# sebadorn/Physically-based-Rendering

Hardware: AMD Instinct MI355X
Metric: Msamples/s (paths/s) @1080p fixed seed; 1/2/4/8 MI355X scaling (higher is better)
Workload: dtype f32

## Files before the change

### physically-based-rendering_amd/csrc/pbr_hip.hip

```cpp
#include <hip/hip_runtime.h>

#include <cmath>
#include <cstdarg>
#include <cstdio>
#include <cstdlib>
#include <cstring>
#include <string>
#include <algorithm>
#include <vector>

#include "pbr_hip.h"
#include "pbr_hip_diag.h"
#include "pt_aux.hpp"
#include "pt_adaptive.hpp"
#include "pt_instances.hpp"
#include "bvh_build.hpp"
#include "pt_denoise.hpp"
#include "pt_scene_pack.hpp"
#include "pt_tuner.hpp"
#include "pt_adaptive_host.hpp"

using ptk::DevParams;

typedef void ( *KernelFn )( const ptk::DevParams );
// ... 91 lines not shown
	bool plansBuilt = false, phongPlanBuilt = false, chainPlansBuilt = false;
	bool workClean = false;
	float* hSeeds = nullptr;
	size_t hSeedCapacity = 0;
	int pinnedPlan = -1;
	char lastPlan[48] = "";
	char lastKernel[96] = "";
	double lastTraceMs = 0.0;
	uint32_t lastTraceLaunches = 0;
	float* dSeeds = nullptr;
	size_t seedCapacity = 0;
	unsigned long long* dCounters = nullptr;
	unsigned int* dWork = nullptr;
	unsigned int* dGuard = nullptr;
	unsigned* dTileFrames = nullptr;
	float* dTileError = nullptr;
	unsigned* dTileActive = nullptr;
	float2* dMoments = nullptr;
	unsigned* dAdaptiveOrder = nullptr;
	hipEvent_t evFoldStart = nullptr, evFoldStop = nullptr;
	bool adaptiveStats = false;
	uint32_t lastAdaptiveRounds = 0;
	uint64_t lastAdaptiveUnits = 0;
	double lastAdaptiveFoldMs = 0.0;
};

namespace {

int fail( pbr_ctx* ctx, int code, const char* fmt, ... ) {
	char buf[512];
	va_list ap;
	va_start( ap, fmt );
	vsnprintf( buf, sizeof( buf ), fmt, ap );
	va_end( ap );

	if( ctx != nullptr ) {
		ctx->error = buf;
	}

	return code;
}

#define HIP_TRY( ctx, call ) \
	do { \
		const hipError_t err__ = ( call ); \
		if( err__ != hipSuccess ) { \
			return fail( ctx, PBR_EDEVICE, "%s: %s", #call, hipGetErrorString( err__ ) ); \
		} \
	} while( 0 )

#define PBR_TRY( call ) \
	do { \
		const int status__ = ( call ); \
		if( status__ != PBR_OK ) { \
			return status__; \
		} \
	} while( 0 )

void freeWalkStreams( pbr_ctx* ctx ) {
	(void) hipFree( ctx->dNodesWalk );
	ctx->dNodesWalk = nullptr;
	ctx->walkBuilt = 0;
	ctx->walkBytes = 0;
}

void freeScene( pbr_ctx* ctx ) {
	(void) hipFree( ctx->dNodes );
	freeWalkStreams( ctx );
	(void) hipFree( ctx->dTris );
	(void) hipFree( ctx->dTriPN );
	ctx->dTriPN = nullptr;
	(void) hipFree( ctx->dFaceN );
	ctx->dFaceN = nullptr;
	(void) hipFree( ctx->dMats );
	(void) hipFree( ctx->dLights );
	ctx->dNodes = ctx->dTris = ctx->dMats = ctx->dLights = nullptr;
	ctx->hasScene = false;
}

void replan( pbr_ctx* ctx ) {
	ctx->plansBuilt = false;
	ctx->chainPlansBuilt = false;
	ctx->phongPlanBuilt = false;
	ctx->tuner.reset( ScheduleTuner::scaleOf( (size_t) ctx->numLocalTiles * 64 ) );
}

void freeImages( pbr_ctx* ctx ) {
	(void) hipFree( ctx->dImgIn );
	(void) hipFree( ctx->dImgOut );
	(void) hipFree( ctx->dImgDbg );
	(void) hipFree( ctx->dRows );
	(void) hipFree( ctx->dFull );
	(void) hipFree( ctx->dFrameBuf );
	ctx->dFrameBuf = nullptr;
	ctx->frameBufFrames = 0;
	(void) hipFree( ctx->dChain );
	ctx->dChain = nullptr;
	ctx->chainFloats = 0;
	(void) hipFree( ctx->dTileOrder );
	(void) hipFree( ctx->dCostOrder );
	(void) hipFree( ctx->dLastOrder );
	ctx->dLastOrder = nullptr;
	ctx->hLastOrder.clear();
	(void) hipFree( ctx->dTileCost );
	(void) hipFree( ctx->dTileFrames );
	(void) hipFree( ctx->dTileError );
	(void) hipFree( ctx->dTileActive );
	(void) hipFree( ctx->dMoments );
	(void) hipFree( ctx->dAdaptiveOrder );
	ctx->dTileFrames = ctx->dTileActive = ctx->dAdaptiveOrder = nullptr;
	ctx->dTileError = nullptr;
	ctx->dMoments = nullptr;
	ctx->adaptiveStats = false;
	ctx->dTileOrder = ctx->dCostOrder = nullptr;
	ctx->dTileCost = nullptr;
	ctx->hTileOrder.clear();
	ctx->hCostOrder.clear();
	ctx->costLearnt = false;
	ctx->orderPinned = false;
	ctx->dImgIn = ctx->dImgOut = ctx->dImgDbg = ctx->dRows = ctx->dFull = nullptr;
	ctx->configured = false;
}

const size_t kWorkBytes = sizeof( unsigned int ) * ( PT_HEADS + 1 ) * PT_BAND_STRIDE;

const size_t kFrameBufBytes = (size_t) 16 << 30;

const size_t kCounterSlots = 16;


#define PTI_DECLARE( f, g ) extern "C" const void* PTI_NAME( f, g )( uint32_t, int, int ) __attribute__( ( weak ) );
#define PTI_DECLARE_FLAVOUR( f ) \
	PTI_DECLARE( f, 0 ) PTI_DECLARE( f, 1 ) PTI_DECLARE( f, 2 ) PTI_DECLARE( f, 3 ) PTI_DECLARE( f, 4 ) PTI_DECLARE( f, 5 ) PTI_DECLARE( f, 6 ) PTI_DECLARE( f, 7 ) \
	PTI_DECLARE( f, 8 )
PTI_DECLARE_FLAVOUR( 0 )
PTI_DECLARE_FLAVOUR( 1 )
PTI_DECLARE_FLAVOUR( 2 )
PTI_DECLARE_FLAVOUR( 3 )
PTI_DECLARE_FLAVOUR( 5 )
PTI_DECLARE_FLAVOUR( 7 )
PTI_DECLARE_FLAVOUR( 8 )
PTI_DECLARE_FLAVOUR( 9 )
PTI_DECLARE_FLAVOUR( 10 )
PTI_DECLARE_FLAVOUR( 11 )
PTI_DECLARE_FLAVOUR( 13 )
PTI_DECLARE_FLAVOUR( 15 )
#define PTI_ROW( f ) { PTI_NAME( f, 0 ), PTI_NAME( f, 1 ), PTI_NAME( f, 2 ), PTI_NAME( f, 3 ), PTI_NAME( f, 4 ), PTI_NAME( f, 5 ), PTI_NAME( f, 6 ), PTI_NAME( f, 7 ), PTI_NAME( f, 8 ) }
#define PTI_NO_ROW { nullptr, nullptr, nullptr, nullptr, nullptr, nullptr, nullptr, nullptr, nullptr }
const pti_picker kPickers[PTI_FLAVOURS][PTI_GROUPS] = { PTI_ROW( 0 ), PTI_ROW( 1 ), PTI_ROW( 2 ), PTI_ROW( 3 ), PTI_NO_ROW, PTI_ROW( 5 ), PTI_NO_ROW, PTI_ROW( 7 ),
                                                       PTI_ROW( 8 ), PTI_ROW( 9 ), PTI_ROW( 10 ), PTI_ROW( 11 ), PTI_NO_ROW, PTI_ROW( 13 ), PTI_NO_ROW, PTI_ROW( 15 ) };

KernelFn pickKernel( int flavour, int group, uint32_t brdf, bool shadow, bool lights ) {
	const pti_picker pick = kPickers[flavour][group];
	return ( pick != nullptr ) ? (KernelFn) pick( brdf, shadow ? 1 : 0, lights ? 1 : 0 ) : nullptr;
}

int flavourOf( uint32_t traversal, uint32_t arith ) {
	return ( ( traversal != 0 ) ? 1 : 0 ) | ( ( arith != 0 ) ? 2 : 0 ) | ( ( traversal == PBR_WALK_EIGHT_ORDERS_COMPACT ) ? 4 : 0 );
}

int flavourOf( const pbr_config& cfg ) {
	return flavourOf( cfg.traversal, cfg.arith );
}

bool dualIsDual( int flavour );

// ... 309 lines not shown
	const size_t slotBytes = spec.pathSlotBytes;

	if( share < slotBytes + 32 ) {
		return fail( ctx, PBR_ESTATE, "plan %s: %zu B of per-lane path state do not fit a block's %zu B share of LDS at %d blocks per CU", spec.name, slotBytes, share, blocksPerCU );
	}

	size_t slots = ( share - slotBytes ) / 32;
	slots = std::min<size_t>( slots, hotAvail );

	if( knobs.ldsSlots >= 0 ) {
		slots = std::min<size_t>( slots, (size_t) knobs.ldsSlots );
	}
	if( flavour & 4 ) {
		slots &= ~(size_t) 1;
	}

	HIP_TRY( ctx, hipFuncSetAttribute( (const void*) kernel, hipFuncAttributeMaxDynamicSharedMemorySize, (int) share ) );

	plan->kernel = kernel;
	plan->blockThreads = spec.blockThreads;
	plan->blocks = ctx->numCUs * blocksPerCU;
	plan->numHot = (int) slots;
	plan->ldsBytes = slots * 32 + slotBytes;
	plan->park = spec.park;
	plan->shade = spec.shade;
	plan->parkEighths = ( ctx->numNodes >= kWideMinNodes ) ? 4 : 6;
	plan->refillBatch = ( knobs.refillBatch >= 1 ) ? std::min( 64, knobs.refillBatch ) : ( ( ctx->numNodes >= kWideMinNodes ) ? kRefillBatchLarge : kRefillBatchSmall );
	plan->drainMode = ( knobs.drainMode >= 0 ) ? knobs.drainMode : 1;

	if( knobs.phPark >= 0 ) {
		plan->park = std::max( 1, std::min( ( spec.pathSlotBytes != 0 ) ? 128 : 64, knobs.phPark ) );
	}
	if( knobs.phShade >= 0 ) {
		plan->shade = std::max( 1, std::min( 64, knobs.phShade ) );
	}
	if( knobs.parkEighths >= 0 ) {
		plan->parkEighths = std::min( 8, knobs.parkEighths );
	}

	plan->name = spec.name;
	const char* const tf[2] = { "false", "true" };
	const int minw[PTI_GROUPS] = { 4, 6, 8, 4, 4, 6, 8, 0, 0 };

	if( spec.group == PTI_DUAL ) {
		std::snprintf( plan->kernelName, sizeof( plan->kernelName ), "ptk_f%d::pathTracingDual<%u, %s, %s>", flavour, ctx->cfg.brdf, tf[shadow], tf[lights] );
	}
	else if( spec.group >= PTI_PHASED_LEAN ) {
		std::snprintf( plan->kernelName, sizeof( plan->kernelName ), "ptk_f%d::pathTracingPhased<%u, %s, %s, %d>", flavour, ctx->cfg.brdf, tf[shadow], tf[lights], minw[spec.group] );
	}
	else {
		std::snprintf( plan->kernelName, sizeof( plan->kernelName ), "ptk_f%d::pathTracing<%u, %s, %s, %d, %s>", flavour, ctx->cfg.brdf, tf[shadow], tf[lights], minw[spec.group], tf[spec.group == PTI_REFILL_PHONG] );
	}

	return PBR_OK;
}

int buildPlans( pbr_ctx* ctx, uint32_t hotAvail, bool phong, bool chained ) {
	if( !ctx->plansBuilt || ( chained && !ctx->chainPlansBuilt ) ) {
		const int flavour = flavourOf( ctx->cfg );
		const bool orderedWalk = ( flavour & 1 ) != 0;
		const PlanSpec specs[ScheduleTuner::kPlans] = {
			{ PTI_REFILL_LEAN, "refill-lean", 0, 0 },
			{ PTI_REFILL_WIDE, "refill-wide", 0, 0 },
			{ PTI_PHASED_LEAN, "phased-lean", 16, 32 },
			{ PTI_PHASED_WIDE, "phased-wide", 16, 48 },
			{ PTI_PHASED_MID, "phased-mid", orderedWalk ? 12 : 16, orderedWalk ? 48 : 40, kMidBlockThreads },
			{ PTI_REFILL_MID, "refill-mid", 0, 0, kMidBlockThreads },
			dualIsDual( flavour ) ? PlanSpec{ PTI_DUAL, "phased-dual", 28, 48, PBR_BLOCK, (size_t) 2 * 4 * 16 * PBR_BLOCK }
			                      : PlanSpec{ PTI_PHASED_MID, "phased-dual", 16, 40, kMidBlockThreads },
		};

		for( int k = 0; k < ScheduleTuner::kPlans; k++ ) {
			if( !ctx->plansBuilt ) {
				PBR_TRY( makePlan( ctx, specs[k], hotAvail, &ctx->plans[k] ) );
				ctx->tuner.names[k] = specs[k].name;
			}
			if( chained && !ctx->chainPlansBuilt ) {
				PBR_TRY( makePlan( ctx, specs[k], hotAvail, &ctx->chainPlans[k], true ) );
			}
		}

		ctx->chainPlansBuilt = ctx->chainPlansBuilt || chained;

		ctx->tuner.log = ( ctx->knobs.tuneLog > 0 ) ? stderr : nullptr;
		ctx->phongPlanBuilt = ctx->plansBuilt && ctx->phongPlanBuilt;
		ctx->plansBuilt = true;
	}

	if( phong && !ctx->phongPlanBuilt ) {
		PBR_TRY( makePlan( ctx, PlanSpec{ PTI_REFILL_PHONG, "refill-lean-phong", 0, 0 }, hotAvail, &ctx->phongPlan ) );
		ctx->phongPlanBuilt = true;
	}

	return PBR_OK;
}

int runPlan( pbr_ctx* ctx, const Plan& plan, DevParams* P, size_t waveUnits ) {
	const size_t wavesPerBlock = (size_t) plan.blockThreads / 64;
	const size_t needed = std::max<size_t>( 1, ( waveUnits + wavesPerBlock - 1 ) / wavesPerBlock );
	const unsigned blocks = (unsigned) std::min<size_t>( (size_t) plan.blocks, needed );
	P->numHot = plan.numHot;
	P->numHotBytes = plan.numHot * 32;
	P->slotBase = plan.numHot * 32;
	P->phPark = plan.park;
	P->phShade = plan.shade;
	P->refillBatch = plan.refillBatch;
	P->drainMode = plan.drainMode;
	P->parkEighths = plan.parkEighths;
	hipLaunchKernelGGL( plan.kernel, dim3( blocks ), dim3( (unsigned) plan.blockThreads ), plan.ldsBytes, ctx->stream, *P );
	HIP_TRY( ctx, hipGetLastError() );
	return PBR_OK;
}

int stageSeeds( pbr_ctx* ctx, const float* seeds, uint32_t nFrames ) {
	if( ctx->seedCapacity < nFrames ) {
		(void) hipFree( ctx->dSeeds );
		ctx->dSeeds = nullptr;
		ctx->seedCapacity = 0;
		HIP_TRY( ctx, hipMalloc( (void**) &ctx->dSeeds, sizeof( float ) * nFrames ) );
		ctx->seedCapacity = nFrames;
	}

	if( ctx->hSeedCapacity < nFrames ) {
		(void) hipHostFree( ctx->hSeeds );
		ctx->hSeeds = nullptr;
		ctx->hSeedCapacity = 0;
		HIP_TRY( ctx, hipHostMalloc( (void**) &ctx->hSeeds, sizeof( float ) * std::max<size_t>( nFrames, 64 ), hipHostMallocDefault ) );
		ctx->hSeedCapacity = std::max<size_t>( nFrames, 64 );
	}

	std::memcpy( ctx->hSeeds, seeds, sizeof( float ) * nFrames );
	HIP_TRY( ctx, hipMemcpyAsync( ctx->dSeeds, ctx->hSeeds, sizeof( float ) * nFrames, hipMemcpyHostToDevice, ctx->stream ) );
	return PBR_OK;
}

int growFrameBuf( pbr_ctx* ctx, uint32_t nFrames, size_t* chunkCap ) {
	const size_t pixelSlots = (size_t) ctx->numLocalTiles * 64;
	const size_t frameBytes = sizeof( float4 ) * pixelSlots;
	const size_t capFrames = std::max<size_t>( 1, kFrameBufBytes / frameBytes );
	size_t cap = std::min<size_t>( capFrames, nFrames );
	cap = std::min<size_t>( cap, std::max<size_t>( 1, 0x7FFFFFFFull / ( pixelSlots + 64 * (size_t) ctx->queueWidth ) ) );

	if( ctx->knobs.chunkFrames >= 1 ) {
		cap = std::min<size_t>( cap, (size_t) ctx->knobs.chunkFrames );
	}

	*chunkCap = cap;

	if( ctx->frameBufFrames < cap ) {
		const size_t frames = std::min<size_t>( capFrames, std::max<size_t>( 256, ( cap <= 256 ) ? cap : 2 * cap ) );
		(void) hipFree( ctx->dFrameBuf );
		ctx->dFrameBuf = nullptr;
		ctx->frameBufFrames = 0;
		HIP_TRY( ctx, hipMalloc( (void**) &ctx->dFrameBuf, frameBytes * frames ) );
		ctx->frameBufFrames = frames;
	}

	return PBR_OK;
}

void dealOrder( pbr_ctx* ctx, uint32_t nFrames, bool settled, DevParams* P ) {
	const Knobs& knobs = ctx->knobs;
	int dealt = 0;

	if( !ctx->orderPinned && ctx->costLearnt && knobs.dealOrder != 0 && ( settled || knobs.dealOrder > 0 ) ) {
		const size_t tileFrames = (size_t) ctx->numLocalTiles * nFrames;
// ... 77 lines not shown
	if( !ctx->hasScene || !ctx->configured ) {
		return fail( ctx, PBR_ESTATE, "render before pbr_upload_scene / pbr_configure" );
	}
	if( cam == nullptr || seeds == nullptr || nFrames == 0 ) {
		return fail( ctx, PBR_EINVAL, "render: null camera / seeds or zero frames" );
	}
	if( ctx->cfg.brdf != ctx->sceneBrdf ) {
		return fail( ctx, PBR_EINVAL, "configured BRDF %u does not match the uploaded materials (BRDF %u)", ctx->cfg.brdf, ctx->sceneBrdf );
	}

	const bool dof = ( cam->focusPoint[0] >= 0 && cam->focusPoint[1] >= 0 );

	if( dof && nFrames > 1 && !chained ) {
		return fail( ctx, PBR_EINVAL, "depth of field reads the previous frame of another pixel: render one frame per call" );
	}
	if( dof && ctx->cfg.tile_world > 1 && !ctx->focusGiven ) {
		return fail( ctx, PBR_EINVAL, "depth of field with tile sharding: the focus pixel's tile may live on another rank — pass its previous-frame distance with pbr_set_focus_depth (owner: pbr_get_focus_depth) before every %s", chained ? "pbr_render_dof call" : "frame" );
	}

	const bool chain = dof && chained;
	ctx->lastChainMs = 0.0;

	HIP_TRY( ctx, hipSetDevice( ctx->device ) );

	for( int k = 0; k < 4; k++ ) {
		( (volatile unsigned*) ctx->dGuard )[k] = 0u;
	}

	PBR_TRY( stageSeeds( ctx, seeds, nFrames ) );

	if( !ctx->workClean ) {
		HIP_TRY( ctx, hipMemsetAsync( ctx->dWork, 0, kWorkBytes, ctx->stream ) );
	}

	ctx->workClean = false;

	DevParams P;
	uint32_t hotAvail = 0;
	PBR_TRY( sceneParams( ctx, &P, &hotAvail ) );
	P.triPN = ctx->dTriPN;
	P.phongAlpha = ctx->cfg.phong_tessellation;
	P.imgIn = ctx->dImgIn;
	P.imgOut = ctx->dImgOut;
	P.imgDbg = ctx->dImgDbg;
	P.counters = ctx->dCounters;
	P.workCounter = ctx->dWork;
	setCamera( &P, cam, (int) ctx->cfg.width, (int) ctx->cfg.height, pxDim );
	P.aperture = cam->lense[0] / cam->lense[1];
	P.samplesF = (float) ctx->cfg.samples;
	P.focusX = cam->focusPoint[0];
	P.focusY = cam->focusPoint[1];
	P.focusGiven = ( dof && ctx->focusGiven ) ? 1 : 0;
	P.focusDepth = ctx->focusDepth;
	ctx->focusGiven = false;
	P.lenseFocal = cam->lense[0];
	P.lenseAperture = cam->lense[1];
	P.tilesX = ctx->tilesX;
	invariantDivisor( (unsigned) ctx->tilesX, P.tilesXDiv );
	P.numLocalTiles = ctx->numLocalTiles;
	P.tileWorld = (int) ctx->cfg.tile_world;
	P.tileRank = (int) ctx->cfg.tile_rank;
	P.maxDepth = (int) ctx->cfg.max_depth;
	P.maxAddedDepth = (int) ctx->cfg.max_added_depth;
	P.samples = (int) ctx->cfg.samples;
	P.useExplicitWeight = explicitWeight ? 1 : 0;
	P.explicitWeight = weight;
	P.antiAliasing = ctx->cfg.anti_aliasing;
	P.sky[0] = ctx->cfg.sky_light[0];
	P.sky[1] = ctx->cfg.sky_light[1];
	P.sky[2] = ctx->cfg.sky_light[2];

	const bool phong = ( ctx->cfg.phong_tessellation > 0.0f );

	if( phong && chain ) {
		return fail( ctx, PBR_EINVAL, "pbr_render_dof does not render Phong tessellation with a focus point (its plan has an intersection of its own); call pbr_render_frame + pbr_accumulate per frame" );
	}
	if( phong && ctx->dTriPN == nullptr ) {
		return fail( ctx, PBR_EINVAL, "Phong tessellation needs a scene with usable vertex normals" );
	}

	PBR_TRY( buildPlans( ctx, hotAvail, phong, chain ) );
	size_t chunkCap = 0;
	PBR_TRY( growFrameBuf( ctx, nFrames, &chunkCap ) );
	ctx->tuner.beginRender( nFrames );

	const Plan* plans = chain ? ctx->chainPlans : ctx->plans;
	const Plan* forced = phong ? &ctx->phongPlan : ( ctx->pinnedPlan >= 0 ) ? &plans[std::min( ScheduleTuner::kPlans - 1, ctx->pinnedPlan )] : nullptr;
	dealOrder( ctx, nFrames, forced != nullptr || ctx->tuner.settled(), &P );
	P.frameBuf = ctx->dFrameBuf;
	const size_t pixelSlots = (size_t) ctx->numLocalTiles * 64;
	P.frameStride = (unsigned) pixelSlots;
	const unsigned foldBlocks = (unsigned) ( ( pixelSlots + 255 ) / 256 );
	double traceMs = 0.0, chainMs = 0.0;
	uint32_t launches = 0, largest = 0;
	HIP_TRY( ctx, hipEventRecord( ctx->evStart, ctx->stream ) );

	for( uint32_t done = 0; done < nFrames; ) {
		const uint32_t most = std::min<uint32_t>( (uint32_t) chunkCap, nFrames - done );
		const Chunk chunk = ( forced != nullptr ) ? Chunk{ -1, most, -1, false } : ctx->tuner.next( most );
		const Plan& plan = ( forced != nullptr ) ? *forced : plans[chunk.plan];
		const uint32_t n = chunk.frames;
		P.nFrames = (int) n;
		invariantDivisor( n, P.framesDiv );
		P.firstCount = (int) ( firstCount + done );
		P.seeds = ctx->dSeeds + done;

		if( chain ) {
			HIP_TRY( ctx, hipEventRecord( ctx->evChainStart, ctx->stream ) );
			PBR_TRY( runFocusChain( ctx, &P, done == 0 ? ctx->dImgIn : ctx->dImgOut, done == 0 ) );
		}

		HIP_TRY( ctx, hipEventRecord( ctx->evTraceStart, ctx->stream ) );
		PBR_TRY( runPlan( ctx, plan, &P, (size_t) ctx->numLocalTiles * n ) );
		HIP_TRY( ctx, hipEventRecord( ctx->evTraceStop, ctx->stream ) );
		hipLaunchKernelGGL( ptk::foldFrames, dim3( foldBlocks ), dim3( 256 ), 0, ctx->stream, P,
			(const float4*) ( done == 0 ? ctx->dImgIn : ctx->dImgOut ), ctx->dImgOut );
		HIP_TRY( ctx, hipGetLastError() );
		HIP_TRY( ctx, hipStreamSynchronize( ctx->stream ) );

		float ms = 0.0f;
		HIP_TRY( ctx, hipEventElapsedTime( &ms, ctx->evTraceStart, ctx->evTraceStop ) );
		traceMs += (double) ms;
		launches++;

		if( chain ) {
			float chainPart = 0.0f;
			HIP_TRY( ctx, hipEventElapsedTime( &chainPart, ctx->evChainStart, ctx->evTraceStart ) );
			chainMs += (double) chainPart;
		}

		if( n > largest ) {
			largest = n;
			std::snprintf( ctx->lastPlan, sizeof( ctx->lastPlan ), "%s", plan.name );
			std::snprintf( ctx->lastKernel, sizeof( ctx->lastKernel ), "%s", plan.kernelName );
		}

		ctx->tuner.record( chunk, (double) ms );
		done += n;
	}

	HIP_TRY( ctx, hipEventRecord( ctx->evStop, ctx->stream ) );
	HIP_TRY( ctx, hipStreamSynchronize( ctx->stream ) );
	ctx->workClean = true;

	float ms = 0.0f;
	HIP_TRY( ctx, hipEventElapsedTime( &ms, ctx->evStart, ctx->evStop ) );
	ctx->lastKernelMs = (double) ms;
	ctx->lastTraceMs = traceMs;
	ctx->lastChainMs = chainMs;
	ctx->lastTraceLaunches = launches;
	ctx->launchesSinceLearn += launches;
	PBR_TRY( checkGuard( ctx ) );
	return learnTileCosts( ctx, cam, pxDim );
}


int adaptiveDealTable( const pbr_ctx* ctx, size_t tiles, uint32_t frames ) {
	const Knobs& knobs = ctx->knobs;

	if( ctx->orderPinned || !ctx->costLearnt || knobs.dealOrder == 0 ) {
		return 0;
	}

	const size_t tileFrames = tiles * frames;
	const size_t costLimit = ( ctx->cfg.tile_world > 1u ) ? kCostOrderShardTileFrames : kCostOrderTileFrames;
	return ( knobs.dealOrder > 0 ) ? std::min( knobs.dealOrder, 2 ) : ( tileFrames <= costLimit ) ? 1 : ( tileFrames <= kSpatialOrderTileFrames ) ? 0 : 2;
}

int launchAdaptive( pbr_ctx* ctx, uint32_t firstCount, const float* seeds, float pxDim, const pbr_camera* cam, const pbr_adaptive_params& A ) {
	if( !ctx->hasScene || !ctx->configured ) {
		return fail( ctx, PBR_ESTATE, "render before pbr_upload_scene / pbr_configure" );
	}
	if( ctx->cfg.brdf != ctx->sceneBrdf ) {
		return fail( ctx, PBR_EINVAL, "configured BRDF %u does not match the uploaded materials (BRDF %u)", ctx->cfg.brdf, ctx->sceneBrdf );
	}

	const bool phong = ( ctx->cfg.phong_tessellation > 0.0f );

	if( phong && ctx->dTriPN == nullptr ) {
		return fail( ctx, PBR_EINVAL, "Phong tessellation needs a scene with usable vertex normals" );
	}

	HIP_TRY( ctx, hipSetDevice( ctx->device ) );
	const size_t tiles = (size_t) ctx->numLocalTiles;
	const size_t pixelSlots = tiles * 64;

	if( ctx->dMoments == nullptr ) {
		HIP_TRY( ctx, hipMalloc( (void**) &ctx->dTileFrames, sizeof( unsigned ) * std::max<size_t>( 1, tiles ) ) );
		HIP_TRY( ctx, hipMalloc( (void**) &ctx->dTileError, sizeof( float ) * std::max<size_t>( 1, tiles ) ) );
		HIP_TRY( ctx, hipMalloc( (void**) &ctx->dTileActive, sizeof( unsigned ) * std::max<size_t>( 1, tiles ) ) );
		HIP_TRY( ctx, hipMalloc( (void**) &ctx->dAdaptiveOrder, sizeof( unsigned ) * std::max<size_t>( 1, tiles ) ) );
		HIP_TRY( ctx, hipMalloc( (void**) &ctx->dMoments, sizeof( float2 ) * std::max<size_t>( 1, pixelSlots ) ) );
	}

	ctx->adaptiveStats = false;
	ctx->lastChainMs = 0.0;

	for( int k = 0; k < 4; k++ ) {
		( (volatile unsigned*) ctx->dGuard )[k] = 0u;
	}

	PBR_TRY( stageSeeds( ctx, seeds, A.max_frames ) );

	if( !ctx->workClean ) {
		HIP_TRY( ctx, hipMemsetAsync( ctx->dWork, 0, kWorkBytes, ctx->stream ) );
	}

	ctx->workClean = false;

	DevParams P;
	uint32_t hotAvail = 0;
	PBR_TRY( sceneParams( ctx, &P, &hotAvail ) );
	P.triPN = ctx->dTriPN;
	P.phongAlpha = ctx->cfg.phong_tessellation;
	P.imgIn = ctx->dImgIn;
	P.imgOut = ctx->dImgOut;
	P.imgDbg = ctx->dImgDbg;
	P.counters = ctx->dCounters;
	P.workCounter = ctx->dWork;
	setCamera( &P, cam, (int) ctx->cfg.width, (int) ctx->cfg.height, pxDim );
// ... 1500 lines not shown
```

### physically-based-rendering_amd/csrc/pt_tuner.hpp

```cpp
#pragma once

#include <algorithm>
#include <cstddef>
#include <cstdint>
#include <cstdio>
#include <cstring>

struct Chunk {
	int plan;
	uint32_t frames;
	int finalist;
	bool screening;
};

class ScheduleTuner {
public:
	static constexpr int kPlans = 7;

	static uint32_t scaleOf( size_t localPixels ) {
		const size_t reference = (size_t) 1920 * 1080;
		const size_t scale = ( reference + localPixels / 2 ) / std::max<size_t>( localPixels, 1 );
		return (uint32_t) std::min<size_t>( std::max<size_t>( scale, 1 ), 64 );
	}

	FILE* log = nullptr;
	const char* names[kPlans] = {};

	void reset( uint32_t scale ) {
		scale_ = scale;
		tuned_ = -1;
		renderFrames_ = tunedAt_ = 0;
		std::memset( screen_, 0, sizeof( screen_ ) );
		finalists_ = 0;
		restartRefinement();
	}

	void beginRender( uint32_t nFrames ) {
		renderFrames_ = std::max( renderFrames_, nFrames );

		if( tuned_ >= 0 && finalists_ > 0 && nFrames > kReevaluateRatio * tunedAt_ ) {
			const Decision again = decide( nFrames );

			if( again.separable ) {
				tuned_ = again.plan;
				tunedAt_ = nFrames;
			}
			else if( nFrames >= kRetimeLongChunks * refineLong() ) {
				tuned_ = -1;
				restartRefinement();
			}
		}
	}

	bool settled() const { return tuned_ >= 0; }
	int tunedPlan() const { return tuned_; }

	Chunk next( uint32_t maxFrames ) const {
		if( tuned_ >= 0 ) {
			return Chunk{ tuned_, maxFrames, -1, false };
		}

		if( finalists_ > 0 ) {
			const uint32_t k = refineChunks_ % (uint32_t) finalists_;
			const uint32_t pass = refineChunks_ / (uint32_t) finalists_;
			const int finalist = ( ( pass & 1u ) != 0u ) ? finalists_ - 1 - (int) k : (int) k;
			const bool longPass = ( pass % kRefinePasses == 1u || pass % kRefinePasses == 2u );
			return Chunk{ finalist_[finalist], std::min<uint32_t>( maxFrames, longPass ? refineLong() : refineShort() ), finalist, false };
		}

		int plan = 0;

		while( plan < kPlans - 1 && screened( plan ) ) {
			plan++;
		}

		return Chunk{ plan, std::min<uint32_t>( maxFrames, screenFrames() - screen_[plan].frames ), -1, true };
	}

	void record( const Chunk& c, double ms ) {
		if( !c.screening && c.finalist < 0 ) {
			return;
		}

		const uint32_t n = c.frames;

		if( log != nullptr ) {
			std::fprintf( log, "[pbr tune] %s %-12s %u frame(s) %.3f ms = %.3f ms/frame\n", c.screening ? "screen" : "refine", names[c.plan], n, ms, ms / n );
		}

		if( c.screening ) {
			screen_[c.plan].ms += ms;
			screen_[c.plan].frames += n;
			screen_[c.plan].launches++;

			if( screened( kPlans - 1 ) ) {
				chooseFinalists();
			}

			return;
		}

		double* fit = fit_[c.finalist];
		fit[0] += 1.0;
		fit[1] += (double) n;
		fit[2] += (double) n * (double) n;
		fit[3] += ms;
		fit[4] += (double) n * ms;
		refineChunks_++;

		if( refineChunks_ >= rounds_ * kRefinePasses * (uint32_t) finalists_ ) {
			const Decision best = decide( renderFrames_ );

			if( best.runnerUp > 0.0 && best.runnerUp < kCloseCall && rounds_ < kMaxRounds ) {
				rounds_ = kMaxRounds;
			}
			else {
				tuned_ = best.plan;
				tunedAt_ = renderFrames_;
			}
		}
	}

	bool fit( int plan, double* a, double* b ) const {
		for( int k = 0; k < finalists_; k++ ) {
			double aFit, bFit;

			if( finalist_[k] == plan && solve( fit_[k], &aFit, &bFit ) && aFit >= 0.0 && bFit >= 0.0 ) {
				*a = aFit;
				*b = bFit;
				return true;
			}
		}

		return false;
	}

	uint32_t budgetFrames() const {
		return (uint32_t) kPlans * screenFrames() + kMaxRounds * (uint32_t) kMaxFinalists * ( kRefinePasses / 2u ) * ( refineShort() + refineLong() );
	}

private:
	static constexpr uint32_t kScreenFrames = 2, kScreenLaunches = 2;
	static constexpr int kMinFinalists = 2, kMaxFinalists = 3;
	static constexpr double kFinalistMargin = 1.10;
	static constexpr uint32_t kRefineShort = 4, kRefineLong = 12, kRefinePasses = 4;
	static constexpr double kCloseCall = 1.05;
	static constexpr uint32_t kMaxRounds = 2;
	static constexpr uint32_t kReevaluateRatio = 2, kRetimeLongChunks = 4;

	uint32_t screenFrames() const { return kScreenFrames * scale_; }
	uint32_t refineShort() const { return kRefineShort * scale_; }
	uint32_t refineLong() const { return kRefineLong * scale_; }

	bool screened( int plan ) const {
		return screen_[plan].frames >= screenFrames() || screen_[plan].launches >= kScreenLaunches;
	}

	void restartRefinement() {
		refineChunks_ = 0;
		rounds_ = 1;
		std::memset( fit_, 0, sizeof( fit_ ) );
	}

	void chooseFinalists() {
		auto perFrame = [&]( int k ) { return screen_[k].ms / screen_[k].frames; };
		int order[kPlans] = { 0, 1, 2, 3, 4, 5, 6 };
		std::sort( order, order + kPlans, [&]( int x, int y ) { return perFrame( x ) < perFrame( y ); } );
		finalists_ = 0;

		for( int k = 0; k < kPlans; k++ ) {
			if( k < kMinFinalists || ( k < kMaxFinalists && perFrame( order[k] ) <= kFinalistMargin * perFrame( order[0] ) ) ) {
				finalist_[finalists_++] = order[k];
			}
		}
	}

	static bool solve( const double f[5], double* a, double* b ) {
		const double det = f[0] * f[2] - f[1] * f[1];

		if( !( det > 1e-9 * f[2] * f[0] ) ) {
			return false;
		}

		*b = ( f[0] * f[4] - f[1] * f[3] ) / det;
		*a = ( f[3] - *b * f[1] ) / f[0];
		return true;
	}

	struct Decision { int plan; bool separable; double runnerUp; };
	Decision decide( uint32_t renderFrames ) const {
		const double frames = (double) std::max<uint32_t>( renderFrames, 1u );
		int best = -1;
		double bestCost = 0.0, secondCost = 0.0;
		bool separable = true;

		for( int k = 0; k < finalists_; k++ ) {
			const double* f = fit_[k];
			double a = 0.0, b = f[3] / f[1], aFit, bFit;
			const bool solved = solve( f, &aFit, &bFit );
			separable = separable && solved;

			if( solved && aFit >= 0.0 && bFit >= 0.0 ) {
				a = aFit;
				b = bFit;
			}

			const double cost = ( a + b * frames ) / frames;

			if( log != nullptr ) {
				std::fprintf( log, "[pbr tune] fit %-12s a %.3f ms  b %.3f ms/frame  -> %.4f ms/frame at %u frames\n", names[finalist_[k]], a, b, cost, (unsigned) frames );
			}

			if( best < 0 || cost < bestCost ) {
				secondCost = ( best < 0 ) ? 0.0 : bestCost;
				best = k;
				bestCost = cost;
			}
			else if( secondCost == 0.0 || cost < secondCost ) {
				secondCost = cost;
			}
		}

		return Decision{ finalist_[best], separable, ( bestCost > 0.0 && secondCost > 0.0 ) ? secondCost / bestCost : 0.0 };
	}

	uint32_t scale_ = 1;
	int tuned_ = -1;
	uint32_t renderFrames_ = 0;
	uint32_t tunedAt_ = 0;
	struct { double ms; uint32_t frames, launches; } screen_[kPlans] = {};
	int finalists_ = 0;
	int finalist_[kMaxFinalists] = {};
	uint32_t refineChunks_ = 0;
	uint32_t rounds_ = 1;
	double fit_[kMaxFinalists][5] = {};
};
```

Measured before the change: 2247.

## Settle close tuner calls with a timed duel and skip unavailable dual plan

When the tuner's linear fits leave finalists within noise or within the close-call margin, it now runs a duel. Production-length chunks of the close plans are timed in palindromic order until the means separate by three sigmas or the frame budget is spent. The tile deal order switches to the settled ordering during the duel, and tile costs are learnt first if needed. It also drops the phased-dual plan from screening when the dual flavour is unavailable, since it then only duplicates phased-mid. The aim is to pick the truly faster schedule and avoid screening a redundant plan, at the cost of more tuning frames run on possibly slower plans.

```diff
diff --git a/physically-based-rendering_amd/csrc/pbr_hip.hip b/physically-based-rendering_amd/csrc/pbr_hip.hip
--- a/physically-based-rendering_amd/csrc/pbr_hip.hip
+++ b/physically-based-rendering_amd/csrc/pbr_hip.hip
@@ -197,6 +197,7 @@
 	ctx->plansBuilt = false;
 	ctx->chainPlansBuilt = false;
 	ctx->phongPlanBuilt = false;
+	ctx->tuner.closeCalls = ScheduleTuner::kDuel;
 	ctx->tuner.reset( ScheduleTuner::scaleOf( (size_t) ctx->numLocalTiles * 64 ) );
 }
 
@@ -672,6 +673,8 @@
 
 		ctx->chainPlansBuilt = ctx->chainPlansBuilt || chained;
 
+		const uint32_t all = ( 1u << ScheduleTuner::kPlans ) - 1u;
+		ctx->tuner.setCandidates( dualIsDual( flavour ) ? all : all & ~( 1u << 6 ) );
 		ctx->tuner.log = ( ctx->knobs.tuneLog > 0 ) ? stderr : nullptr;
 		ctx->phongPlanBuilt = ctx->plansBuilt && ctx->phongPlanBuilt;
 		ctx->plansBuilt = true;
@@ -915,11 +918,12 @@
 	PBR_TRY( buildPlans( ctx, hotAvail, phong, chain ) );
 	size_t chunkCap = 0;
 	PBR_TRY( growFrameBuf( ctx, nFrames, &chunkCap ) );
-	ctx->tuner.beginRender( nFrames );
+	ctx->tuner.beginRender( nFrames, (uint32_t) std::min<size_t>( chunkCap, 0xFFFFFFFFu ) );
 
 	const Plan* plans = chain ? ctx->chainPlans : ctx->plans;
 	const Plan* forced = phong ? &ctx->phongPlan : ( ctx->pinnedPlan >= 0 ) ? &plans[std::min( ScheduleTuner::kPlans - 1, ctx->pinnedPlan )] : nullptr;
-	dealOrder( ctx, nFrames, forced != nullptr || ctx->tuner.settled(), &P );
+	bool dealtAsSettled = ( forced != nullptr || ctx->tuner.settled() );
+	dealOrder( ctx, nFrames, dealtAsSettled, &P );
 	P.frameBuf = ctx->dFrameBuf;
 	const size_t pixelSlots = (size_t) ctx->numLocalTiles * 64;
 	P.frameStride = (unsigned) pixelSlots;
@@ -933,6 +937,15 @@
 		const Chunk chunk = ( forced != nullptr ) ? Chunk{ -1, most, -1, false } : ctx->tuner.next( most );
 		const Plan& plan = ( forced != nullptr ) ? *forced : plans[chunk.plan];
 		const uint32_t n = chunk.frames;
+
+		if( chunk.duel != dealtAsSettled && forced == nullptr && !ctx->tuner.settled() ) {
+			if( chunk.duel && !ctx->costLearnt && ( launches > 0 || ctx->launchesSinceLearn > 0 ) ) {
+				PBR_TRY( learnTileCosts( ctx, cam, pxDim ) );
+			}
+
+			dealtAsSettled = chunk.duel;
+			dealOrder( ctx, nFrames, dealtAsSettled, &P );
+		}
 		P.nFrames = (int) n;
 		invariantDivisor( n, P.framesDiv );
 		P.firstCount = (int) ( firstCount + done );
@@ -968,7 +981,7 @@
 			std::snprintf( ctx->lastKernel, sizeof( ctx->lastKernel ), "%s", plan.kernelName );
 		}
 
-		ctx->tuner.record( chunk, (double) ms );
+		ctx->tuner.record( chunk, (double) ms, ctx->lastDeal );
 		done += n;
 	}
 
diff --git a/physically-based-rendering_amd/csrc/pt_tuner.hpp b/physically-based-rendering_amd/csrc/pt_tuner.hpp
--- a/physically-based-rendering_amd/csrc/pt_tuner.hpp
+++ b/physically-based-rendering_amd/csrc/pt_tuner.hpp
@@ -1,6 +1,7 @@
 #pragma once
 
 #include <algorithm>
+#include <cmath>
 #include <cstddef>
 #include <cstdint>
 #include <cstdio>
@@ -11,6 +12,7 @@
 	uint32_t frames;
 	int finalist;
 	bool screening;
+	bool duel;
 };
 
 class ScheduleTuner {
@@ -25,6 +27,13 @@
 
 	FILE* log = nullptr;
 	const char* names[kPlans] = {};
+
+	enum CloseCalls { kSecondPalindrome, kDuel };
+	CloseCalls closeCalls = kSecondPalindrome;
+
+	void setCandidates( uint32_t mask ) {
+		candidates_ = mask & ( ( 1u << kPlans ) - 1u );
+	}
 
 	void reset( uint32_t scale ) {
 		scale_ = scale;
@@ -33,10 +42,16 @@
 		std::memset( screen_, 0, sizeof( screen_ ) );
 		finalists_ = 0;
 		restartRefinement();
-	}
-
-	void beginRender( uint32_t nFrames ) {
+		spent_ = 0;
+	}
+
+	void beginRender( uint32_t nFrames, uint32_t chunkCap = 0xFFFFFFFFu ) {
 		renderFrames_ = std::max( renderFrames_, nFrames );
+		chunkCap_ = std::max<uint32_t>( chunkCap, 1u );
+
+		if( duellists_ > 0 && std::min( nFrames, chunkCap_ ) < duelLength_ ) {
+			settleDuel( "the calls became shorter than its chunks" );
+		}
 
 		if( tuned_ >= 0 && finalists_ > 0 && nFrames > kReevaluateRatio * tunedAt_ ) {
 			const Decision again = decide( nFrames );
@@ -57,7 +72,18 @@
 
 	Chunk next( uint32_t maxFrames ) const {
 		if( tuned_ >= 0 ) {
-			return Chunk{ tuned_, maxFrames, -1, false };
+			return Chunk{ tuned_, maxFrames, -1, false, false };
+		}
+
+		if( duellists_ > 0 ) {
+			if( maxFrames < duelLength_ ) {
+				return Chunk{ finalist_[duelLeader()], maxFrames, -1, false, true };
+			}
+
+			const uint32_t k = duelChunks_ % (uint32_t) duellists_;
+			const uint32_t pass = duelChunks_ / (uint32_t) duellists_;
+			const int finalist = duellist_[( ( pass & 1u ) != 0u ) ? duellists_ - 1 - (int) k : (int) k];
+			return Chunk{ finalist_[finalist], duelLength_, finalist, false, true };
 		}
 
 		if( finalists_ > 0 ) {
@@ -65,7 +91,7 @@
 			const uint32_t pass = refineChunks_ / (uint32_t) finalists_;
 			const int finalist = ( ( pass & 1u ) != 0u ) ? finalists_ - 1 - (int) k : (int) k;
 			const bool longPass = ( pass % kRefinePasses == 1u || pass % kRefinePasses == 2u );
-			return Chunk{ finalist_[finalist], std::min<uint32_t>( maxFrames, longPass ? refineLong() : refineShort() ), finalist, false };
+			return Chunk{ finalist_[finalist], std::min<uint32_t>( maxFrames, longPass ? refineLong() : refineShort() ), finalist, false, false };
 		}
 
 		int plan = 0;
@@ -74,15 +100,21 @@
 			plan++;
 		}
 
-		return Chunk{ plan, std::min<uint32_t>( maxFrames, screenFrames() - screen_[plan].frames ), -1, true };
-	}
-
-	void record( const Chunk& c, double ms ) {
+		return Chunk{ plan, std::min<uint32_t>( maxFrames, screenFrames() - screen_[plan].frames ), -1, true, false };
+	}
+
+	void record( const Chunk& c, double ms, const char* dealt = "" ) {
+		if( c.duel ) {
+			recordDuel( c, ms, dealt );
+			return;
+		}
+
 		if( !c.screening && c.finalist < 0 ) {
 			return;
 		}
 
 		const uint32_t n = c.frames;
+		spent_ += n;
 
 		if( log != nullptr ) {
 			std::fprintf( log, "[pbr tune] %s %-12s %u frame(s) %.3f ms = %.3f ms/frame\n", c.screening ? "screen" : "refine", names[c.plan], n, ms, ms / n );
@@ -93,7 +125,7 @@
 			screen_[c.plan].frames += n;
 			screen_[c.plan].launches++;
 
-			if( screened( kPlans - 1 ) ) {
+			if( allScreened() ) {
 				chooseFinalists();
 			}
 
@@ -106,12 +138,18 @@
 		fit[2] += (double) n * (double) n;
 		fit[3] += ms;
 		fit[4] += (double) n * ms;
+		fit[5] += ms * ms;
 		refineChunks_++;
 
 		if( refineChunks_ >= rounds_ * kRefinePasses * (uint32_t) finalists_ ) {
-			const Decision best = decide( renderFrames_ );
-
-			if( best.runnerUp > 0.0 && best.runnerUp < kCloseCall && rounds_ < kMaxRounds ) {
+			double costs[kMaxFinalists];
+			const Decision best = decide( renderFrames_, costs );
+			const bool close = ( best.runnerUp > 0.0 && ( best.runnerUp < kCloseCall || ( closeCalls == kDuel && withinTheFitsNoise( renderFrames_, costs ) ) ) );
+
+			if( close && closeCalls == kDuel ) {
+				startDuel( best.plan, costs );
+			}
+			else if( close && rounds_ < kMaxRounds ) {
 				rounds_ = kMaxRounds;
 			}
 			else {
@@ -136,8 +174,17 @@
 	}
 
 	uint32_t budgetFrames() const {
-		return (uint32_t) kPlans * screenFrames() + kMaxRounds * (uint32_t) kMaxFinalists * ( kRefinePasses / 2u ) * ( refineShort() + refineLong() );
-	}
+		const uint32_t palindrome = (uint32_t) kMaxFinalists * ( kRefinePasses / 2u ) * ( refineShort() + refineLong() );
+		return (uint32_t) kPlans * screenFrames() + palindrome + ( ( closeCalls == kDuel ) ? duelFrames() : ( kMaxRounds - 1u ) * palindrome );
+	}
+
+	uint32_t duelLength( uint32_t renderFrames, uint32_t chunkCap ) const {
+		const uint32_t cap = std::max<uint32_t>( std::min( kDuelCap * scale_, chunkCap ), 1u );
+		const uint32_t n = std::max<uint32_t>( renderFrames, 1u );
+		return n / ( ( n + cap - 1u ) / cap );
+	}
+
+	int duellists() const { return duellists_; }
 
 private:
 	static constexpr uint32_t kScreenFrames = 2, kScreenLaunches = 2;
@@ -146,36 +193,61 @@
 	static constexpr uint32_t kRefineShort = 4, kRefineLong = 12, kRefinePasses = 4;
 	static constexpr double kCloseCall = 1.05;
 	static constexpr uint32_t kMaxRounds = 2;
+	static constexpr uint32_t kDuelCap = 24, kDuelFrames = 256;
+	static constexpr double kDuelSigmas = 3.0;
+	static constexpr double kFitSigmas = 3.0;
 	static constexpr uint32_t kReevaluateRatio = 2, kRetimeLongChunks = 4;
 
 	uint32_t screenFrames() const { return kScreenFrames * scale_; }
 	uint32_t refineShort() const { return kRefineShort * scale_; }
 	uint32_t refineLong() const { return kRefineLong * scale_; }
+	uint32_t duelFrames() const { return kDuelFrames * scale_; }
+
+	bool candidate( int plan ) const { return ( ( candidates_ >> plan ) & 1u ) != 0u; }
 
 	bool screened( int plan ) const {
-		return screen_[plan].frames >= screenFrames() || screen_[plan].launches >= kScreenLaunches;
+		return !candidate( plan ) || screen_[plan].frames >= screenFrames() || screen_[plan].launches >= kScreenLaunches;
+	}
+
+	bool allScreened() const {
+		for( int plan = 0; plan < kPlans; plan++ ) {
+			if( !screened( plan ) ) {
+				return false;
+			}
+		}
+
+		return true;
 	}
 
 	void restartRefinement() {
 		refineChunks_ = 0;
 		rounds_ = 1;
 		std::memset( fit_, 0, sizeof( fit_ ) );
+		duellists_ = 0;
+		spent_ = (uint32_t) kPlans * screenFrames();
 	}
 
 	void chooseFinalists() {
 		auto perFrame = [&]( int k ) { return screen_[k].ms / screen_[k].frames; };
-		int order[kPlans] = { 0, 1, 2, 3, 4, 5, 6 };
-		std::sort( order, order + kPlans, [&]( int x, int y ) { return perFrame( x ) < perFrame( y ); } );
+		int order[kPlans], plans = 0;
+
+		for( int k = 0; k < kPlans; k++ ) {
+			if( candidate( k ) ) {
+				order[plans++] = k;
+			}
+		}
+
+		std::sort( order, order + plans, [&]( int x, int y ) { return perFrame( x ) < perFrame( y ); } );
 		finalists_ = 0;
 
-		for( int k = 0; k < kPlans; k++ ) {
+		for( int k = 0; k < plans; k++ ) {
 			if( k < kMinFinalists || ( k < kMaxFinalists && perFrame( order[k] ) <= kFinalistMargin * perFrame( order[0] ) ) ) {
 				finalist_[finalists_++] = order[k];
 			}
 		}
 	}
 
-	static bool solve( const double f[5], double* a, double* b ) {
+	static bool solve( const double f[6], double* a, double* b ) {
 		const double det = f[0] * f[2] - f[1] * f[1];
 
 		if( !( det > 1e-9 * f[2] * f[0] ) ) {
@@ -188,7 +260,7 @@
 	}
 
 	struct Decision { int plan; bool separable; double runnerUp; };
-	Decision decide( uint32_t renderFrames ) const {
+	Decision decide( uint32_t renderFrames, double* costs = nullptr ) const {
 		const double frames = (double) std::max<uint32_t>( renderFrames, 1u );
 		int best = -1;
 		double bestCost = 0.0, secondCost = 0.0;
@@ -207,6 +279,10 @@
 
 			const double cost = ( a + b * frames ) / frames;
 
+			if( costs != nullptr ) {
+				costs[k] = cost;
+			}
+
 			if( log != nullptr ) {
 				std::fprintf( log, "[pbr tune] fit %-12s a %.3f ms  b %.3f ms/frame  -> %.4f ms/frame at %u frames\n", names[finalist_[k]], a, b, cost, (unsigned) frames );
 			}
@@ -224,7 +300,180 @@
 		return Decision{ finalist_[best], separable, ( bestCost > 0.0 && secondCost > 0.0 ) ? secondCost / bestCost : 0.0 };
 	}
 
+	bool withinTheFitsNoise( uint32_t renderFrames, const double costs[] ) const {
+		const double frames = (double) std::max<uint32_t>( renderFrames, 1u );
+		double rss = 0.0, freedom = 0.0;
+
+		for( int k = 0; k < finalists_; k++ ) {
+			const double* f = fit_[k];
+			double a, b;
+
+			if( !solve( f, &a, &b ) || f[0] <= 2.0 ) {
+				return false;
+			}
+
+			rss += std::max( 0.0, f[5] - a * f[3] - b * f[4] );
+			freedom += f[0] - 2.0;
+		}
+
+		int best = 0, second = -1;
+
+		for( int k = 1; k < finalists_; k++ ) {
+			if( costs[k] < costs[best] ) {
+				second = best;
+				best = k;
+			}
+			else if( second < 0 || costs[k] < costs[second] ) {
+				second = k;
+			}
+		}
+
+		auto variance = [&]( int k ) {
+			const double* f = fit_[k];
+			const double mean = f[1] / f[0], spread = f[2] - f[1] * f[1] / f[0];
+			return ( rss / freedom ) * ( 1.0 / f[0] + ( frames - mean ) * ( frames - mean ) / spread ) / ( frames * frames );
+		};
+
+		return costs[second] - costs[best] < kFitSigmas * std::sqrt( variance( best ) + variance( second ) );
+	}
+
+
+	void startDuel( int fitBest, const double costs[] ) {
+		int best = 0;
+
+		for( int k = 0; k < finalists_; k++ ) {
+			best = ( finalist_[k] == fitBest ) ? k : best;
+		}
+
+		duellists_ = 0;
+		duellist_[duellists_++] = best;
+
+		int second = -1;
+
+		for( int k = 0; k < finalists_; k++ ) {
+			second = ( k != best && ( second < 0 || costs[k] < costs[second] ) ) ? k : second;
+		}
+
+		for( int k = 0; k < finalists_; k++ ) {
+			if( k != best && ( k == second || costs[k] < kCloseCall * costs[best] ) ) {
+				duellist_[duellists_++] = k;
+			}
+		}
+
+		duelLength_ = duelLength( renderFrames_, chunkCap_ );
+		duelChunks_ = duelSpent_ = 0;
+		std::memset( duel_, 0, sizeof( duel_ ) );
+
+		if( log != nullptr ) {
+			std::fprintf( log, "[pbr tune] close call at %u frames: %d plans duel in chunks of %u frames, %u frames at most\n", renderFrames_, duellists_, duelLength_, budgetFrames() - std::min( spent_, budgetFrames() ) );
+		}
+
+		if( spent_ + 2u * (uint32_t) duellists_ * duelLength_ > budgetFrames() ) {
+			duellists_ = 0;
+			tuned_ = fitBest;
+			tunedAt_ = renderFrames_;
+		}
+	}
+
+	int duelLeader() const {
+		int leader = duellist_[0];
+
+		for( int d = 0; d < duellists_; d++ ) {
+			if( duel_[duellist_[d]].n == 0.0 ) {
+				return duellist_[0];
+			}
+		}
+
+		for( int d = 1; d < duellists_; d++ ) {
+			const int k = duellist_[d];
+
+			if( duel_[k].sum / duel_[k].n < duel_[leader].sum / duel_[leader].n ) {
+				leader = k;
+			}
+		}
+
+		return leader;
+	}
+
+	void recordDuel( const Chunk& c, double ms, const char* dealt ) {
+		if( duellists_ == 0 ) {
+			return;
+		}
+
+		duelSpent_ += c.frames;
+		spent_ += c.frames;
+
+		if( c.finalist < 0 ) {
+			if( log != nullptr ) {
+				std::fprintf( log, "[pbr tune] duel   %-12s %u frame(s), the rest of a call: not timed\n", names[c.plan], c.frames );
+			}
+		}
+		else {
+			const double perFrame = ms / c.frames;
+			duel_[c.finalist].n += 1.0;
+			duel_[c.finalist].sum += perFrame;
+			duel_[c.finalist].squares += perFrame * perFrame;
+			duelChunks_++;
+
+			if( log != nullptr ) {
+				std::fprintf( log, "[pbr tune] duel   %-12s %u frame(s) %.3f ms = %.4f ms/frame  dealt %s\n", names[c.plan], c.frames, ms, perFrame, dealt );
+			}
+		}
+
+		const uint32_t palindrome = 2u * (uint32_t) duellists_;
+		const uint32_t under = duelChunks_ % palindrome;
+
+		if( c.finalist >= 0 && under == 0u && separated() ) {
+			settleDuel( "separated" );
+		}
+		else if( spent_ + ( palindrome - under ) * duelLength_ > budgetFrames() ) {
+			settleDuel( "its frames are spent" );
+		}
+	}
+
+	bool separated() const {
+		const int leader = duelLeader();
+		const double n = duel_[leader].n, mean = duel_[leader].sum / n;
+		const double var = std::max( 0.0, duel_[leader].squares - n * mean * mean ) / ( n - 1.0 );
+
+		for( int d = 0; d < duellists_; d++ ) {
+			const int k = duellist_[d];
+
+			if( k == leader ) {
+				continue;
+			}
+
+			const double nK = duel_[k].n, meanK = duel_[k].sum / nK;
+			const double varK = std::max( 0.0, duel_[k].squares - nK * meanK * meanK ) / ( nK - 1.0 );
+
+			if( !( meanK - mean > kDuelSigmas * std::sqrt( var / n + varK / nK ) ) ) {
+				return false;
+			}
+		}
+
+		return true;
+	}
+
+	void settleDuel( const char* why ) {
+		const int leader = duelLeader();
+
+		if( log != nullptr ) {
+			for( int d = 0; d < duellists_; d++ ) {
+				const int k = duellist_[d];
+				std::fprintf( log, "[pbr tune] duel   %-12s mean %.4f ms/frame over %d chunk(s)\n", names[finalist_[k]], ( duel_[k].n > 0.0 ) ? duel_[k].sum / duel_[k].n : 0.0, (int) duel_[k].n );
+			}
+
+			std::fprintf( log, "[pbr tune] duel over (%s) after %u frames: %s\n", why, duelSpent_, names[finalist_[leader]] );
+		}
+
+		tuned_ = finalist_[leader];
+		tunedAt_ = renderFrames_;
+		duellists_ = 0;
+	}
+
 	uint32_t scale_ = 1;
+	uint32_t candidates_ = ( 1u << kPlans ) - 1u;
+	uint32_t chunkCap_ = 0xFFFFFFFFu;
 	int tuned_ = -1;
 	uint32_t renderFrames_ = 0;
 	uint32_t tunedAt_ = 0;
@@ -233,5 +482,11 @@
 	int finalist_[kMaxFinalists] = {};
 	uint32_t refineChunks_ = 0;
 	uint32_t rounds_ = 1;
-	double fit_[kMaxFinalists][5] = {};
+	double fit_[kMaxFinalists][6] = {};
+	uint32_t spent_ = 0;
+	int duellists_ = 0;
+	int duellist_[kMaxFinalists] = {};
+	uint32_t duelLength_ = 0;
+	uint32_t duelChunks_ = 0, duelSpent_ = 0;
+	struct { double n, sum, squares; } duel_[kMaxFinalists] = {};
 };
```

Result: no change. 2240 (-0.3%).
